# CityU-AIM-Group/MultiModal-learning

Measured on AMD Instinct MI355X. Metric: ROI-tiles/sec (teacher+student distill step), higher is better.
Workload: dtype bf16; 1 GPU; BASELINE configs[1]: teacher+student distill step, bf16, batch 64 per GPU, 512x512 tiles, 320-d omic, CRD P=300/K=700->P2=20/K2=512, n_data=1024, GK-Refine on, Adam+EMA, dropout 0.1; tiles_per_gpu=64, tile=512, global_batch=64, parallelism=single, launch=one captured HIP graph per step, input_pipeline=inputs resident in HBM when the timed region starts

## Files before the change

### multimodal-learning_amd/csrc/bn_act.hip

```cpp
#include "ph_common.h"
#include <cstdlib>
#include "ph_kernels.h"

namespace {

template <typename T>
__global__ void pack_input_kernel(const float* __restrict__ x, T* __restrict__ x4, int B, int H, int W) {
  const size_t npix = (size_t)B * H * W;
  const size_t i = (size_t)blockIdx.x * blockDim.x + threadIdx.x;
  if (i >= npix) return;
  const size_t hw = (size_t)H * W;
  const size_t b = i / hw, r = i - b * hw;
  const float c0 = x[(b * 3 + 0) * hw + r], c1 = x[(b * 3 + 1) * hw + r], c2 = x[(b * 3 + 2) * hw + r];
  if constexpr (is_hp<T>::value) {
    f16x4 h, l;
    f16 a, b;
    hp_split(c0, a, b); h[0] = a; l[0] = b;
    hp_split(c1, a, b); h[1] = a; l[1] = b;
    hp_split(c2, a, b); h[2] = a; l[2] = b;
    h[3] = (f16)0.f; l[3] = (f16)0.f;
    f16* base = reinterpret_cast<f16*>(x4);
    *reinterpret_cast<f16x4*>(base + i * 4) = h;
    *reinterpret_cast<f16x4*>(base + (npix + i) * 4) = l;
  } else if constexpr (is_f32<T>::value) {
// ... 42 lines not shown
  }
}

__global__ void bn_eval_params_kernel(PhBnEvalTable t, float eps) {
  const int u = blockIdx.x;
  for (int c = threadIdx.x; c < t.C[u]; c += blockDim.x) {
    const float is = rsqrtf(t.running_var[u][c] + eps);
    const float sc = t.gamma[u][c] * is;
    t.mean[u][c] = t.running_mean[u][c];
    t.invstd[u][c] = is;
    t.scale[u][c] = sc;
    t.shift[u][c] = t.beta[u][c] - t.running_mean[u][c] * sc;
  }
}

template <typename T, typename TY>
__global__ void bn_apply_kernel(const TY* __restrict__ y, const float* __restrict__ scale,
                                const float* __restrict__ shift, const TY* __restrict__ res,
                                const TY* __restrict__ y_r, const float* __restrict__ scale_r,
                                const float* __restrict__ shift_r, T* __restrict__ out, TY* __restrict__ out32, size_t n8,
                                int C8, int relu, int res_as_t) {
  const size_t i0 = (size_t)blockIdx.x * blockDim.x + threadIdx.x;
  if (i0 >= n8) return;
  const size_t gstride = (size_t)gridDim.x * blockDim.x;
  const int c = (int)(i0 % C8) * 8;
  const bool use_res = res != nullptr, use_yr = !use_res && y_r != nullptr;
  auto fetch = [&](size_t i, float (&v)[8], float (&r)[8]) {
    load8(y + i * 8, v);
    if (use_res) {
      if (!std::is_same<T, TY>::value && res_as_t) load8(reinterpret_cast<const T*>(res) + i * 8, r);
      else load8(res + i * 8, r);
    } else if (use_yr) {
      load8(y_r + i * 8, r);
    }
  };
  float v[8], r[8];
// ... 25 lines not shown
          const float t = __builtin_fmaf(r[k], scr8[k], shr8[k]);
          if constexpr (is_hp<T>::value) v[k] += (t > 0.f ? t : 0.f);
          else v[k] += (float)(T)(t > 0.f ? t : 0.f);
        }
      } else {
#pragma unroll
        for (int k = 0; k < 8; ++k) v[k] += r[k] * scr8[k] + shr8[k];
      }
    }
    if (relu & 1) {
#pragma unroll
      for (int k = 0; k < 8; ++k) v[k] = v[k] > 0.f ? v[k] : 0.f;
    }
    store8(out + i * 8, v);
    if constexpr (!std::is_same<T, TY>::value) { if (out32) store8(out32 + i * 8, v); }
    if (!more) break;
#pragma unroll
    for (int k = 0; k < 8; ++k) { v[k] = vn[k]; r[k] = rn[k]; }
    i = inext;
  }
}

template <typename T, typename TY, bool IDX>
__global__ void bn_relu_maxpool_kernel(const TY* __restrict__ y, const float* __restrict__ scale,
                                       const float* __restrict__ shift, T* __restrict__ out,
                                       uint8_t* __restrict__ idx, TY* __restrict__ raw, TY* __restrict__ out32, int B, int H,
                                       int W, int C8) {
  const int OH = (H + 1) / 2, OW = (W + 1) / 2;
  const size_t n = (size_t)B * OH * OW * C8;
  const size_t i = (size_t)blockIdx.x * blockDim.x + threadIdx.x;
// ... 116 lines not shown
  __device__ __forceinline__ void get(size_t i8, int c, float (&dz)[8], float (&yy)[8]) const {
    load8(g + i8 * 8, dz);
    load8(y + i8 * 8, yy);
    if (a) {
      float m[8];
      load8(a + i8 * 8, m);
#pragma unroll
      for (int k = 0; k < 8; ++k) dz[k] = m[k] > 0.f ? dz[k] : 0.f;
    } else if (mscale) {
#pragma unroll
      for (int k = 0; k < 8; ++k) dz[k] = __builtin_fmaf(yy[k], mscale[c + k], mshift[c + k]) > 0.f ? dz[k] : 0.f;
    }
  }
};

constexpr int BWD_BLOCKS_MAX = 1024;

template <typename T, typename Src>
__global__ __launch_bounds__(256) void bn_bwd_reduce_kernel(Src src, const float* __restrict__ mean,
                                                            const float* __restrict__ invstd,
                                                            float* __restrict__ parts, size_t npix, int C,
                                                            float* __restrict__ amax) {
  const int C8 = C >> 3;
  const int cg = threadIdx.x % C8, pl = threadIdx.x / C8, npl = 256 / C8;
  const int c = cg * 8;
  float mu[8], is[8], s1[8], s2[8], am = 0.f;
#pragma unroll
  for (int k = 0; k < 8; ++k) { s1[k] = 0.f; s2[k] = 0.f; }
  load8(mean + c, mu); load8(invstd + c, is);
  const size_t per = (npix + gridDim.x - 1) / gridDim.x;
// ... 362 lines not shown
  hipLaunchKernelGGL(bn_finalize_kernel, dim3(C), dim3(256), 0, st, parts, nparts, C, count, eps, momentum, gamma, beta,
                     mean, invstd, scale, shift, running_mean, running_var, nbt);
  PH_LAUNCH_CHECK();
  return PH_OK;
}

int ph_bn_eval_params_launch(const PhBnEvalTable* t, float eps, hipStream_t st) {
  hipLaunchKernelGGL(bn_eval_params_kernel, dim3(t->n), dim3(256), 0, st, *t, eps);
  PH_LAUNCH_CHECK();
  return PH_OK;
}

int ph_bn_apply_launch(const void* y, const float* scale, const float* shift, const void* res, const void* y_r,
                       const float* scale_r, const float* shift_r, void* out, void* out32, size_t npix, int C, int relu, int prec,
                       hipStream_t st) {
  return ph_bn_apply_launch2(y, scale, shift, res, y_r, scale_r, shift_r, out, out32, npix, C, relu, prec, 0, st);
}

int ph_bn_apply_launch2(const void* y, const float* scale, const float* shift, const void* res, const void* y_r,
                        const float* scale_r, const float* shift_r, void* out, void* out32, size_t npix, int C, int relu, int prec,
                        int res_as_t, hipStream_t st) {
  const size_t n8 = npix * (C / 8);
  void* tok = nullptr;
  if (ph_prof_on())
    ph_prof_begin(PH_CLS_BN_APPLY, (double)npix * C * (prec == PH_PREC_BF16 ? 2.0 : 4.0) * ((res || y_r) ? 3.0 : 2.0), st, &tok);
#define PH_CALL(T, TY)                                                                                              \
  hipLaunchKernelGGL((bn_apply_kernel<T, TY>), dim3(ew_grid(n8, C / 8)), dim3(256), 0, st, (const TY*)y, scale, shift, (const TY*)res, \
                     (const TY*)y_r, scale_r, shift_r, (T*)out, (TY*)out32, n8, C / 8, relu, res_as_t)
  PH_DISPATCH(prec, PH_CALL);
#undef PH_CALL
  ph_prof_end(tok, st);
  PH_LAUNCH_CHECK();
  return PH_OK;
}

int ph_bn_relu_maxpool_launch(const void* y, const float* scale, const float* shift, void* out, uint8_t* idx, void* raw,
                              void* out32, int B, int H, int W, int C, int prec, hipStream_t st) {
  const int OH = (H + 1) / 2, OW = (W + 1) / 2;
  const size_t n = (size_t)B * OH * OW * (C / 8);
#define PH_CALL(T, TY)                                                                                                          \
  do {                                                                                                                          \
    if (idx) hipLaunchKernelGGL((bn_relu_maxpool_kernel<T, TY, true>), dim3(nblk(n)), dim3(256), 0, st, (const TY*)y, scale, shift, \
                                (T*)out, idx, (TY*)raw, (TY*)out32, B, H, W, C / 8);                                            \
// ... 28 lines not shown
  const size_t n8 = (size_t)B * HW * (C / 8);
#define PH_CALL(T, TY) hipLaunchKernelGGL(avgpool_bwd_kernel<TY>, dim3(nblk(n8)), dim3(256), 0, st, g, (TY*)dx, n8, HW, C / 8, accumulate)
  PH_DISPATCH(prec, PH_CALL);
#undef PH_CALL
  PH_LAUNCH_CHECK();
  return PH_OK;
}

int ph_bn_bwd_parts(size_t npix, int C) {
  const size_t b = (npix * (size_t)(C / 8) + 2047) / 2048;
  return (int)(b < (size_t)BWD_BLOCKS_MAX ? (b ? b : 1) : BWD_BLOCKS_MAX);
}

int ph_bn_bwd_reduce_launch(const void* g, const void* a, const void* y, const float* mean, const float* invstd,
                            float* parts, size_t npix, int C, int prec, const float* mscale, const float* mshift,
                            float* amax, hipStream_t st) {
  const int nb = ph_bn_bwd_parts(npix, C);
#define PH_CALL(T, TY)                                                                                                       \
  do {                                                                                                                       \
    DzPlain<T, TY> s{(const TY*)g, (const TY*)a, (const TY*)y, mscale, mshift};                                              \
    hipLaunchKernelGGL((bn_bwd_reduce_kernel<T, DzPlain<T, TY>>), dim3(nb), dim3(256), 0, st, s, mean, invstd, parts, npix, C, amax); \
  } while (0)
  PH_DISPATCH(prec, PH_CALL);
#undef PH_CALL
  PH_LAUNCH_CHECK();
  return PH_OK;
}

int ph_bn_bwd_finalize_launch(const float* parts, int nparts, int C, double count, float* dgamma, float* dbeta,
                              float* c1, float* c2, const float* amax, int namax, const float* gamma, const float* invstd,
                              float* dzs, hipStream_t st) {
  hipLaunchKernelGGL(bn_bwd_finalize_kernel, dim3(C), dim3(256), 0, st, parts, nparts, C, count, dgamma, dbeta, c1, c2,
// ... 1 lines not shown
  PH_LAUNCH_CHECK();
  return PH_OK;
}

int ph_bn_bwd_finalize_fused_launch(const float* parts, int nparts, int C, double count, float* dgamma, float* dbeta,
                                    float* c1, float* c2, const float* invstd, int row2, hipStream_t st) {
  if (row2 != 1 && row2 != 2) return PH_EINVAL;
  hipLaunchKernelGGL(bn_bwd_finalize_kernel, dim3(C), dim3(256), 0, st, parts, nparts, C, count, dgamma, dbeta, c1, c2,
                     (const float*)nullptr, 0, (const float*)nullptr, invstd, (float*)nullptr, 3, row2, invstd);
  PH_LAUNCH_CHECK();
  return PH_OK;
}

int ph_bn_bwd_apply_launch(const void* g, const void* a, const void* y, const float* mean, const float* invstd,
                           const float* gamma, const float* c1, const float* c2, void* dy, size_t npix, int C,
                           int prec, const float* mscale, const float* mshift, const float* dzs, hipStream_t st) {
  const size_t n8 = npix * (C / 8);
#define PH_CALL(T, TY)                                                                                                       \
  do {                                                                                                                       \
    DzPlain<T, TY> s{(const TY*)g, (const TY*)a, (const TY*)y, mscale, mshift};                                              \
    hipLaunchKernelGGL((bn_bwd_apply_kernel<T, DzPlain<T, TY>>), dim3(ew_grid(n8, C / 8)), dim3(256), 0, st, s, mean, invstd, gamma, c1, c2, \
                       (T*)dy, n8, C / 8, dzs);                                                                              \
  } while (0)
  PH_DISPATCH(prec, PH_CALL);
#undef PH_CALL
  PH_LAUNCH_CHECK();
  return PH_OK;
}

int ph_stem_bwd_parts(int B, int H) { return (B * H + STEM_ROWS - 1) / STEM_ROWS; }

int ph_stem_bwd_reduce_launch(const void* dpool, const uint8_t* idx, const void* y0, const void* raw, const float* mean,
// ... 49 lines not shown
```

### multimodal-learning_amd/csrc/conv_wgrad.hip

```cpp
#include "ph_common.h"
#include "ph_kernels.h"

namespace {

__device__ __forceinline__ void lds_dma16(const void* g, unsigned lds_addr) {
  asm volatile("s_mov_b32 m0, %0\n\ts_nop 0\n\tglobal_load_lds_dwordx4 %1, off" : : "s"(lds_addr), "v"(g) : "memory");
}

__device__ __forceinline__ int sw_piece(int pix, int piece) { return piece ^ (((pix >> 1) & 1) << 1); }

template <typename T, int S, int TH, int KS>
struct WgCfg {
  static constexpr bool SPLIT = is_f32<T>::value;
  static constexpr bool HPM = is_hp<T>::value;
  static constexpr int TW = 16, BM = TH * TW;
  static constexpr int HPH = (TH - 1) * S + KS, HPW = (TW - 1) * S + KS, HP = HPH * HPW;
  static constexpr int HPP = (HP + 7) / 8 * 8;
  static constexpr int D_BYTES = BM * 128, X_BYTES = HPP * 128;
  static constexpr int NP = SPLIT ? PH_NPLANES : 1;
  static constexpr int LDS_BYTES = SPLIT ? (D_BYTES + X_BYTES) * NP : 2 * (D_BYTES + X_BYTES);
  static constexpr int NT = KS * KS;
};

template <typename T>
// ... 28 lines not shown
template <typename T, int S, int TH, int KS>
__global__ __launch_bounds__(256) void wgrad_kernel(PhWgrad p) {
  using C = WgCfg<T, S, TH, KS>;
  constexpr bool SPLIT = C::SPLIT, HPM = C::HPM;
  constexpr int TW = C::TW, BM = C::BM, HPW = C::HPW, HP = C::HP, NT = C::NT, NP = C::NP;
  typedef typename std::conditional<HPM, f16, T>::type TI;
  constexpr int EW = HPM ? 2 : 1;
  extern __shared__ __attribute__((aligned(16))) unsigned char smem[];
  unsigned char* ldsD = smem;
  unsigned char* ldsX = smem + C::D_BYTES * NP;

  const int tid = threadIdx.x, lane = tid & 63;
  const int wave = __builtin_amdgcn_readfirstlane(tid >> 6);
  const int cf = wave >> 1, kf = wave & 1;
  const int cin_blocks = p.Cin >> 6;
  const int co0 = (blockIdx.x / cin_blocks) << 6, ci0 = (blockIdx.x % cin_blocks) << 6;
  const int chunk = blockIdx.y;
  const int tiles_w = (p.OW + TW - 1) / TW, tiles_h = (p.OH + TH - 1) / TH;
  const int tiles_img = tiles_w * tiles_h, ntiles = tiles_img * p.B;
  const int t_begin = chunk * p.tiles_per_chunk;
  const int t_end = min(ntiles, t_begin + p.tiles_per_chunk);
  const TI* X = reinterpret_cast<const TI*>(p.x);
  const TI* DY = reinterpret_cast<const TI*>(p.dy);
  const long xpix = (p.x_pix_stride ? p.x_pix_stride : p.Cin) * EW;
  const long xrow = (p.x_row_stride ? p.x_row_stride : (long)p.IW * p.Cin) * EW;
  const long ximg = (p.x_img_stride ? p.x_img_stride : (long)p.IH * p.IW * p.Cin) * EW;
  const long dpix = (long)p.Cout * EW;

  f32x16 acc[NT];
#pragma unroll
  for (int t = 0; t < NT; ++t)
#pragma unroll
// ... 472 lines not shown
    }
    hipLaunchKernelGGL(pack_all_tiled_hp_kernel<false>, dim3(pt.tstart[t->n]), dim3(256), 0, st, *t, pt, (f16*)packed, 0);
  } else if (tiled && nplanes == 1)
    hipLaunchKernelGGL(pack_all_tiled_kernel<1>, dim3(pt.tstart[t->n]), dim3(256), 0, st, *t, pt, (bf16*)packed);
  else if (tiled && nplanes == 3)
    hipLaunchKernelGGL(pack_all_tiled_kernel<3>, dim3(pt.tstart[t->n]), dim3(256), 0, st, *t, pt, (bf16*)packed);
  else
    hipLaunchKernelGGL(pack_all_kernel, dim3((unsigned)((t->total + 255) / 256)), dim3(256), 0, st, *t, (bf16*)packed,
                       nplanes);
  PH_LAUNCH_CHECK();
  return PH_OK;
}

int ph_wgrad_tile_h(int S) { return S == 1 ? 8 : 4; }

int ph_wgrad_launch(const PhWgrad* p, int prec, hipStream_t st) {
  if (p->Cin % 64 || p->Cout % 64 || p->nchunks < 1) return PH_EINVAL;
  if (prec == PH_PREC_BF16) { ph_dispatch_note(PH_DK_WGRAD_BF16); return launch_wg_T<bf16>(*p, st); }
  if (prec == PH_PREC_FP16X3 || prec == PH_PREC_FP16X1) {
    PhWgrad q = *p;
    q.hp_hi_only = prec == PH_PREC_FP16X1;
    ph_dispatch_note(PH_DK_WGRAD_HP16);
    return launch_wg_T<hp16>(q, st);
  }
  if (PH_IS_SPLIT_PREC(prec)) {
    PhWgrad q = *p;
    q.prod6 = prec == PH_PREC_BF16X6;
    ph_dispatch_note(PH_DK_WGRAD_F32);
    return launch_wg_T<float>(q, st);
  }
  return PH_EINVAL;
}
// ... 30 lines not shown
```

### multimodal-learning_amd/csrc/ph_kernels.h

```cpp
#pragma once
#include <hip/hip_runtime.h>
#include <stdint.h>

#define PH_CLS_TAPCONV_N64 0
#define PH_CLS_TAPCONV_N128 1
#define PH_CLS_TAPCONV_S2 2
#define PH_CLS_WGRAD 3
#define PH_CLS_STEM_FWD 4
#define PH_CLS_STEM_WGRAD 5
#define PH_CLS_TAPCONV2 6
#define PH_CLS_TAPCONV2_RES 7
#define PH_CLS_CRD_SCORE 8
#define PH_CLS_CRD_LOSSGRAD 9
#define PH_CLS_ADAM_EMA 10
#define PH_CLS_BN_APPLY 11
#define PH_CLS_TAPCONV2_MASKED 12
#define PH_CLS_TAPCONV2_FUSEDIN 13
#define PH_CLS_TAPCONV2_RES_FUSEDIN 14
#define PH_CLS_CRD_TOPK 15
#define PH_NCLS 16
#define PH_NUM_CLS 6
bool ph_prof_on();
int ph_num_cus();
void ph_prof_begin(int cls, double work, hipStream_t st, void** token);
// ... 84 lines not shown
int ph_tapconv6b_launch(const PhTapConv* p, hipStream_t st);
int ph_tapconv6b_stat_parts(const PhTapConv* p);
bool ph_tapconv2_setup_s2_fwd(PhTapConv* t, int Cin, int Cout, int IH, int IW, int prec);

struct PhWgrad {
  const void* x;
  const void* dy;
  float* slab;
  const void* zeros;
  int B, IH, IW, Cin, OH, OW, Cout;
  int S, pad, KS;
  int nchunks, tiles_per_chunk;
  long x_pix_stride, x_row_stride, x_img_stride;
  int prod6;
  int hp_hi_only;
};
int ph_wgrad_launch(const PhWgrad* p, int prec, hipStream_t st);
int ph_wgrad_tile_h(int S);
int ph_wgrad_reduce_launch(const float* slab, float* dw_oihw, int nchunks, int KS, int Cout, int Cin, const float* unscale,
                           hipStream_t st);

struct PhStem {
  const void* x4;
  const void* w;
  size_t wplane;
  void* out;
  float* stats;
  int B, IH, IW, OH, OW;
  int prod6;
  int vblocks;
};
// ... 40 lines not shown
                          float* shift, float* running_mean, float* running_var, int64_t* num_batches_tracked,
                          hipStream_t st);
struct PhBnEvalTable {
  const float* gamma[20]; const float* beta[20]; const float* running_mean[20]; const float* running_var[20];
  float* mean[20]; float* invstd[20]; float* scale[20]; float* shift[20];
  int C[20];
  int n;
};
int ph_bn_eval_params_launch(const PhBnEvalTable* t, float eps, hipStream_t st);
int ph_bn_apply_launch(const void* y, const float* scale, const float* shift, const void* res, const void* y_r,
                       const float* scale_r, const float* shift_r, void* out, void* out32, size_t npix, int C, int relu, int prec,
                       hipStream_t st);
int ph_bn_apply_launch2(const void* y, const float* scale, const float* shift, const void* res, const void* y_r,
                        const float* scale_r, const float* shift_r, void* out, void* out32, size_t npix, int C, int relu, int prec,
                        int res_as_t, hipStream_t st);
int ph_avgpool_launch_t(const void* x, float* out, int B, int HW, int C, int prec, hipStream_t st);
int ph_bn_relu_maxpool_launch(const void* y, const float* scale, const float* shift, void* out, uint8_t* idx, void* raw,
                              void* out32, int B, int H, int W, int C, int prec, hipStream_t st);
int ph_avgpool_launch(const void* x, float* out, int B, int HW, int C, int prec, hipStream_t st);
int ph_avgpool_bwd_launch(const float* g, void* dx, int B, int HW, int C, int accumulate, int prec, hipStream_t st);
int ph_bn_bwd_parts(size_t npix, int C);
int ph_stem_bwd_parts(int B, int H);
int ph_bn_bwd_reduce_launch(const void* g, const void* a, const void* y, const float* mean, const float* invstd,
                            float* parts, size_t npix, int C, int prec, const float* mscale, const float* mshift,
                            float* amax, hipStream_t st);
int ph_bn_bwd_finalize_launch(const float* parts, int nparts, int C, double count, float* dgamma, float* dbeta,
                              float* c1, float* c2, const float* amax, int namax, const float* gamma, const float* invstd,
                              float* dzs, hipStream_t st);
int ph_bn_bwd_finalize_fused_launch(const float* parts, int nparts, int C, double count, float* dgamma, float* dbeta,
                                    float* c1, float* c2, const float* invstd, int row2, hipStream_t st);
int ph_bn_bwd_apply_launch(const void* g, const void* a, const void* y, const float* mean, const float* invstd,
                           const float* gamma, const float* c1, const float* c2, void* dy, size_t npix, int C,
                           int prec, const float* mscale, const float* mshift, const float* dzs, hipStream_t st);
int ph_stem_bwd_reduce_launch(const void* dpool, const uint8_t* idx, const void* y0, const void* raw_at_argmax, const float* mean,
                              const float* invstd, const float* scale, const float* shift, float* parts, int B, int H,
                              int W, int C, int prec, float* amax, hipStream_t st);
int ph_stem_bwd_apply_launch(const void* dpool, const uint8_t* idx, const void* y0, const float* mean,
                             const float* invstd, const float* scale, const float* shift, const float* gamma,
                             const float* c1, const float* c2, void* dy0, int B, int H, int W, int C, int prec,
                             const float* dzs, hipStream_t st);
```

### multimodal-learning_amd/csrc/resnet_plan.hip

```cpp
#include <atomic>
#include <cstdlib>
#include <iterator>
#include <mutex>
#include <new>
#include <unordered_map>
#include <vector>
#include "ph_common.h"
#include "ph_kernels.h"
#include "ph_dense.h"

namespace {

struct Unit {
  int Cin, Cout, KS, S, pad;
  int IH, IW, OH, OW;
  size_t wf_off, wd_off;
  size_t wplane;
  size_t y_off;
  size_t st_off;
  mutable int wfrag_f = 0, wfrag_d = 0;
};

void fwd_geometry(const Unit& u, PhTapConv& t) {
  t.IH = u.IH; t.IW = u.IW; t.Cin = u.Cin; t.Cout = u.Cout;
// ... 3 lines not shown
}
void dgrad_s1_geometry(const Unit& u, PhTapConv& t) {
  t.IH = u.OH; t.IW = u.OW; t.Cin = u.Cout; t.Cout = u.Cin;
  t.OH = u.IH; t.OW = u.IW;
  t.OHt = u.IH; t.OWt = u.IW; t.os = 1; t.oa_h = 0; t.oa_w = 0;
  t.iy0 = -(u.KS - 1 - u.pad); t.ix0 = t.iy0; t.ntaps = u.KS * u.KS;
  for (int k = 0; k < t.ntaps; ++k) {
    const int dyy = k / u.KS, dxx = k % u.KS;
    t.dy[k] = dyy; t.dx[k] = dxx; t.wtap[k] = (u.KS - 1 - dyy) * u.KS + (u.KS - 1 - dxx);
  }
}
struct Block {
  int u1, u2, uds;
  size_t in_off, a1_off, out_off;
  size_t in32_off, out32_off;
  int IH, IW, OH, OW, Cin, Cout;
};

constexpr size_t ALIGN = 256;
inline size_t up(size_t x) { return (x + ALIGN - 1) / ALIGN * ALIGN; }

}

struct PhResnetPlan {
  int B, H, W, prec, es;
  std::vector<Unit> units;
  std::vector<Block> blocks;
  size_t x4_off, p0_off, p0raw_off, idx_off, parts_off, parts_bytes;
  size_t g0_off, g1_off, dy_off, da_off, slab_off, slab_bytes, bparts_off, cc_off, zero_off;
  size_t ws_bytes, packed_bytes;
// ... 129 lines not shown
  P->slab_off = take(slab_max);
  {
    const size_t stem_rows = (size_t)ph_stem_bwd_parts(B, s.OH);
    const size_t a = (size_t)1024 * 2 * 512, b = stem_rows * 2 * 64;
    P->bparts_off = take((a > b ? a : b) * sizeof(float));
  }
  P->cc_off = take(2 * 512 * sizeof(float));
  P->zero_off = take(256);
  {
    const size_t rows = std::max((size_t)1024, (size_t)ph_stem_bwd_parts(B, s.OH));
    P->amax_off = take(rows * sizeof(float));
    P->dzs_off = take(256);
  }
  P->fparts_off = take((size_t)1024 * 3 * 512 * sizeof(float));
  P->cc2_off = take(2 * 512 * sizeof(float));
  P->ws_bytes = off;
  P->packed_bytes = woff * sizeof(bf16);
  refresh_layouts(P);
  return P;
}

void ph_resnet_plan_destroy(PhResnetPlan* P) { delete P; }
size_t ph_resnet_workspace_bytes(const PhResnetPlan* P) { return P ? P->ws_bytes : 0; }
size_t ph_resnet_packed_bytes(const PhResnetPlan* P) { return P ? P->packed_bytes : 0; }
int ph_resnet_num_units(const PhResnetPlan* P) { return P ? (int)P->units.size() : 0; }
int ph_resnet_unit_shape(const PhResnetPlan* P, int u, int* out4) {
  if (!P || u < 0 || u >= (int)P->units.size()) return PH_EINVAL;
  out4[0] = P->units[u].Cout; out4[1] = P->units[u].Cin; out4[2] = P->units[u].KS; out4[3] = P->units[u].S;
  return PH_OK;
}
// ... 64 lines not shown
  }
  int rc = ph_tapconv_launch(&t, S, P->prec, c.st);
  if (rc || c.eval) return rc;
  const int nparts = ph_tapconv_stat_parts(&t, S, P->prec);
  float* rm = c.update_running ? (float*)c.params[ui * 6 + 3] : nullptr;
  return ph_bn_finalize_launch(t.stats, nparts, u.Cout, (double)P->B * u.OH * u.OW, 1e-5f, 0.1f,
                               (const float*)c.params[ui * 6 + 1], (const float*)c.params[ui * 6 + 2], c.stat(u, 0),
                               c.stat(u, 1), c.stat(u, 2), c.stat(u, 3), rm, (float*)c.params[ui * 6 + 4],
                               (int64_t*)c.params[ui * 6 + 5], c.st);
}

struct Bst { int u = -1, u2 = -1; const void* a = nullptr; };

int bst_switch(int set) {
  static int on = [] { const char* e = getenv("PH_BST"); return (e && e[0] == '0') ? 0 : 1; }();
  if (set >= 0) on = set ? 1 : 0;
  return on;
}

int conv_dgrad(const Ctx& c, int ui, const void* dy, void* dx, const void* res_g, const void* res_a, const float* dzs = nullptr,
               const Bst* bst = nullptr, int* fused_parts = nullptr) {
  const PhResnetPlan* P = c.P;
  const Unit& u = P->units[ui];
  PhTapConv t{};
  t.in = dy; t.w = c.pk + u.wd_off; t.wplane = u.wplane; t.in_unscale = dzs;
  t.out = dx; t.stats = nullptr; t.res_g = res_g; t.res_a = res_a;
  t.B = P->B; t.IH = u.OH; t.IW = u.OW; t.Cin = u.Cout; t.Cout = u.Cin;
  t.OH = u.IH; t.OW = u.IW;
  t.w_frag = u.wfrag_d;
  if (fused_parts) *fused_parts = 0;
// ... 81 lines not shown
  w.x = x; w.dy = dy; w.slab = reinterpret_cast<float*>(c.ws + P->slab_off);
  w.zeros = c.ws + P->zero_off;
  w.B = P->B; w.IH = u.IH; w.IW = u.IW; w.Cin = u.Cin; w.OH = u.OH; w.OW = u.OW; w.Cout = u.Cout;
  w.S = u.S; w.pad = u.pad; w.KS = u.KS;
  if (u.KS == 1 && u.S == 2) {
    w.x_pix_stride = 2L * u.Cin; w.x_row_stride = 2L * u.IW * u.Cin; w.x_img_stride = (long)u.IH * u.IW * u.Cin;
    w.IH = u.OH; w.IW = u.OW; w.S = 1;
  }
  w.nchunks = wgrad_chunks(u, P->B, &w.tiles_per_chunk, c.wg_want);
  int rc = ph_wgrad_launch(&w, c.bprec(), c.st);
  if (rc) return rc;
  return ph_wgrad_reduce_launch(w.slab, dw, w.nchunks, u.KS, u.Cout, u.Cin, dzs, c.st);
}

int bn_bwd(const Ctx& c, int ui, const void* g, const void* a, void* dy, float* dgamma, float* dbeta, bool self_mask = false,
           float* dzs = nullptr, int fused_parts = 0, int row2 = 1, bool cc2 = false, bool finalize = true, bool apply = true) {
  const PhResnetPlan* P = c.P;
  const Unit& u = P->units[ui];
  const size_t npix = (size_t)P->B * u.OH * u.OW;
  float* parts = reinterpret_cast<float*>(c.ws + P->bparts_off);
  float* c1 = reinterpret_cast<float*>(c.ws + (cc2 ? P->cc2_off : P->cc_off));
  float* c2 = c1 + 512;
  const void* y = c.ws + u.y_off;
  const float* ms = self_mask ? c.stat(u, 2) : nullptr;
  const float* mh = self_mask ? c.stat(u, 3) : nullptr;
  if (self_mask) a = nullptr;
  float* amax = dzs ? c.amax() : nullptr;
  int rc = PH_OK;
  if (finalize) {
    if (fused_parts > 0) {
      rc = ph_bn_bwd_finalize_fused_launch(reinterpret_cast<const float*>(c.ws + P->fparts_off), fused_parts, u.Cout, (double)npix,
                                           dgamma, dbeta, c1, c2, c.stat(u, 1), row2, c.st);
    } else {
      const int nparts = ph_bn_bwd_parts(npix, u.Cout);
      rc = ph_bn_bwd_reduce_launch(g, a, y, c.stat(u, 0), c.stat(u, 1), parts, npix, u.Cout, P->prec, ms, mh, amax, c.st);
      if (rc) return rc;
      rc = ph_bn_bwd_finalize_launch(parts, nparts, u.Cout, (double)npix, dgamma, dbeta, c1, c2, amax, nparts,
                                     (const float*)c.params[ui * 6 + 1], c.stat(u, 1), dzs, c.st);
    }
    if (rc) return rc;
  }
  if (!apply) return PH_OK;
  return ph_bn_bwd_apply_launch(g, a, y, c.stat(u, 0), c.stat(u, 1), (const float*)c.params[ui * 6 + 1], c1, c2, dy, npix,
                                u.Cout, P->prec, ms, mh, dzs, c.st);
}

}

extern "C" {

int ph_resnet_forward(const PhResnetPlan* P, const void* const* params, const void* packed, const float* x_nchw,
                      void* ws_, float* f3, float* f4, int flags, hipStream_t st) {
  if (!P || !params || !packed || !x_nchw || !ws_) return PH_EINVAL;
  Ctx c{P, params, reinterpret_cast<const bf16*>(packed), reinterpret_cast<unsigned char*>(ws_), st,
        (flags & 2) ? 0 : (flags & 1), (flags & 2) ? 1 : 0};
  P->no_masked = (flags & 16) ? 1 : 0;
  c.no_masked = P->no_masked;
  unsigned char* ws = c.ws;
  const bool hp = P->prec == PH_PREC_FP16X3;
// ... 57 lines not shown
                                    (int64_t*)params[5], st)))
      return rc;
    if ((rc = ph_bn_relu_maxpool_launch(ws + u.y_off, c.stat(u, 2), c.stat(u, 3), ws + P->p0_off,
                                        (flags & 4) ? nullptr : ws + P->idx_off, (flags & 4) ? nullptr : ws + P->p0raw_off,
                                        (hp && !fo_hp) ? ws + P->blocks[0].in32_off : nullptr, P->B, u.OH, u.OW, 64, P->prec, st)))
      return rc;
  }
  const bool fuse_a1 = (flags & 4) && !(flags & 8) && P->prec == PH_PREC_BF16;
  for (size_t bi = 0; bi < P->blocks.size(); ++bi) {
    const Block& b = P->blocks[bi];
    const Unit& u1 = P->units[b.u1];
    const Unit& u2 = P->units[b.u2];
    const size_t npix = (size_t)P->B * b.OH * b.OW;
    const Unit& u0 = P->units[0];
    const bool raw_in = bi == 0 && p0_raw;
    if ((rc = raw_in ? conv_fwd(c, b.u1, ws + b.in_off, c.stat(u0, 2), c.stat(u0, 3)) : conv_fwd(c, b.u1, ws + b.in_off))) return rc;
    static const bool fuse_all = [] { const char* e = getenv("PH_FUSE_ALL"); return e && e[0] == '1'; }();
    if (fuse_a1 && (b.Cout <= 128 || fuse_all)) {
      if ((rc = conv_fwd(c, b.u2, ws + u1.y_off, c.stat(u1, 2), c.stat(u1, 3)))) return rc;
    } else {
      if ((rc = ph_bn_apply_launch(ws + u1.y_off, c.stat(u1, 2), c.stat(u1, 3), nullptr, nullptr, nullptr, nullptr,
                                   ws + b.a1_off, nullptr, npix, b.Cout, 1, P->prec, st)))
        return rc;
      if ((rc = conv_fwd(c, b.u2, ws + b.a1_off))) return rc;
    }
    if (b.uds >= 0) {
      const Unit& ud = P->units[b.uds];
      if ((rc = conv_fwd(c, b.uds, ws + b.in_off))) return rc;
      rc = ph_bn_apply_launch(ws + u2.y_off, c.stat(u2, 2), c.stat(u2, 3), nullptr, ws + ud.y_off, c.stat(ud, 2),
                              c.stat(ud, 3), ws + b.out_off, (hp && !fo_hp) ? ws + b.out32_off : nullptr, npix, b.Cout, 1, P->prec, st);
    } else {
      rc = raw_in ? ph_bn_apply_launch(ws + u2.y_off, c.stat(u2, 2), c.stat(u2, 3), nullptr, ws + b.in_off, c.stat(u0, 2),
                                       c.stat(u0, 3), ws + b.out_off, nullptr, npix, b.Cout, 3, P->prec, st)
                  : ph_bn_apply_launch2(ws + u2.y_off, c.stat(u2, 2), c.stat(u2, 3), fo_hp ? ws + b.in_off : ws + b.in32_off, nullptr,
                                        nullptr, nullptr, ws + b.out_off, (hp && !fo_hp) ? ws + b.out32_off : nullptr, npix, b.Cout, 1,
                                        P->prec, fo_hp ? 1 : 0, st);
    }
    if (rc) return rc;
    if ((bi == 5 && f3) || (bi == 7 && f4)) {
      float* dst = bi == 5 ? f3 : f4;
      if ((rc = fo_hp ? ph_avgpool_launch_t(ws + b.out_off, dst, P->B, b.OH * b.OW, b.Cout, P->prec, st)
                      : ph_avgpool_launch(ws + b.out32_off, dst, P->B, b.OH * b.OW, b.Cout, P->prec, st)))
        return rc;
    }
  }
  return PH_OK;
}

}

namespace {
// ... 127 lines not shown
  if (part != 1) {
    if (hipMemsetAsync(ws + P->zero_off, 0, 256, st) != hipSuccess) return PH_ELAUNCH;
    const Block& b = P->blocks[7];
    PH_STAGE(ph_avgpool_bwd_launch(g_f4, gcur, P->B, b.OH * b.OW, b.Cout, 0, P->prec, st));
  }
  for (int bi = bi_hi; bi >= bi_lo; --bi) {
    const Block& b = P->blocks[bi];
    if (bi == 5 && g_f3) {
      PH_STAGE(ph_avgpool_bwd_launch(g_f3, gcur, P->B, b.OH * b.OW, b.Cout, 1, P->prec, st));
      fused_out = 0;
    }
    const void* out = ws + b.out32_off;
    const void* a1 = ws + b.a1_off;
    const void* xin = ws + b.in_off;
    const void* xin32 = ws + b.in32_off;
    if ((rc = claim(k))) return rc;
    if (fused_out > 0 && b.uds >= 0 &&
        (rc = bn_bwd(c, b.uds, gcur, out, nullptr, (float*)grads[b.uds * 3 + 1], (float*)grads[b.uds * 3 + 2], false, nullptr,
                     fused_out, 2, true, true, false)))
      return rc;
    const bool ds_done = fused_out > 0 && b.uds >= 0;
    PH_STAGE(bn_bwd(c, b.u2, gcur, out, dzb[k], (float*)grads[b.u2 * 3 + 1], (float*)grads[b.u2 * 3 + 2], false, c.dzs(k), fused_out));
    fused_out = 0;
    if (!ov) PH_STAGE(wgrad_of(b.u2, a1, k));
    int fused_a1 = 0;
    {
      Bst bs; bs.u = b.u1;
      PH_STAGE(conv_dgrad(c, b.u2, dzb[k], dab, nullptr, nullptr, c.dzs(k), &bs, &fused_a1));
    }
    if (ov) PH_STAGE(wgrad_of(b.u2, a1, k));
    k ^= 1;
    if ((rc = claim(k))) return rc;
    PH_STAGE(bn_bwd(c, b.u1, dab, a1, dzb[k], (float*)grads[b.u1 * 3 + 1], (float*)grads[b.u1 * 3 + 2], true, c.dzs(k), fused_a1));
    if (!ov) PH_STAGE(wgrad_of(b.u1, xin, k));
    if (b.uds < 0) {
      Bst bs;
      if (bi > bi_lo) {
        const Block& pb = P->blocks[bi - 1];
        bs.u = pb.u2; bs.u2 = pb.uds; bs.a = xin32;
      }
        PH_STAGE(conv_dgrad(c, b.u1, dzb[k], gnext, gcur, out, c.dzs(k), &bs, &fused_out));
      if (ov) PH_STAGE(wgrad_of(b.u1, xin, k));
      k ^= 1;
    } else {
        PH_STAGE(conv_dgrad(c, b.u1, dzb[k], gnext, nullptr, nullptr, c.dzs(k)));
      if (ov) PH_STAGE(wgrad_of(b.u1, xin, k));
      k ^= 1;
      if ((rc = claim(k))) return rc;
      PH_STAGE(bn_bwd(c, b.uds, gcur, out, dzb[k], (float*)grads[b.uds * 3 + 1], (float*)grads[b.uds * 3 + 2], false, c.dzs(k),
                      0, 1, ds_done, !ds_done));
      if (!ov) PH_STAGE(wgrad_of(b.uds, xin, k));
        PH_STAGE(conv_dgrad(c, b.uds, dzb[k], gnext, gnext, nullptr, c.dzs(k)));
      if (ov) PH_STAGE(wgrad_of(b.uds, xin, k));
      k ^= 1;
    }
    unsigned char* t = gcur; gcur = gnext; gnext = t;
  }
  if (part != 0) {
    const Unit& u = P->units[0];
    const size_t npix = (size_t)P->B * u.OH * u.OW;
    float* parts = reinterpret_cast<float*>(ws + P->bparts_off);
    float* c1 = reinterpret_cast<float*>(ws + P->cc_off);
    float* c2 = c1 + 512;
    if ((rc = ph_stem_bwd_reduce_launch(gcur, ws + P->idx_off, ws + u.y_off, ws + P->p0raw_off, c.stat(u, 0), c.stat(u, 1),
                                        c.stat(u, 2), c.stat(u, 3), parts, P->B, u.OH, u.OW, 64, P->prec, c.amax(), st)))
// ... 32 lines not shown

}

extern "C" {

unsigned long long ph_resnet_plan_layout_sig(const PhResnetPlan* P) { return P ? refresh_layouts(P) : 0; }

int ph_resnet_plan_set_backward_prec(const PhResnetPlan* P, int prec) {
  if (!P || (prec != -1 && P->prec == PH_PREC_BF16)) return PH_EINVAL;
  if (prec != -1 && !(P->prec == PH_PREC_FP16X3 ? (prec == PH_PREC_FP16X1 || prec == PH_PREC_FP16X3) : PH_IS_SPLIT_PREC(prec))) return PH_EINVAL;
  P->bwd_prec = prec;
  return PH_OK;
}

int ph_debug_set_bst(int on) { return bst_switch(on ? 1 : 0); }

int ph_resnet_plan_set_backward_overlap(const PhResnetPlan* P, int on) {
  if (!P) return PH_EINVAL;
  P->bwd_overlap = on ? 1 : 0;
  return PH_OK;
}

int ph_pack_input(const float* x_nchw, void* x4, int B, int H, int W, int prec, hipStream_t st) {
  if (!x_nchw || !x4 || B < 1 || H < 1 || W < 1 || (prec != PH_PREC_BF16 && !PH_IS_SPLIT_PREC(prec) && prec != PH_PREC_FP16X3))
    return PH_EINVAL;
  return ph_pack_input_launch(x_nchw, x4, B, H, W, prec, st);
}

int ph_resnet_backward(const PhResnetPlan* P, const void* const* params, const void* packed, void* ws_,
                       const float* g_f3, const float* g_f4, void* const* grads, hipStream_t st) {
// ... 18 lines not shown
  Ctx c{P, params, reinterpret_cast<const bf16*>(packed), reinterpret_cast<unsigned char*>(ws_), st, 0, 1};
  c.no_masked = P->no_masked;
  unsigned char* ws = c.ws;
  unsigned char* gcur = ws + P->g0_off;
  unsigned char* gnext = ws + P->g1_off;
  unsigned char* dyb = ws + P->dy_off;
  unsigned char* dab = ws + P->da_off;
  float* c1 = reinterpret_cast<float*>(ws + P->cc_off);
  float* c2 = c1 + 512;
  int rc;
  if (hipMemsetAsync(ws + P->zero_off, 0, 256, st) != hipSuccess) return PH_ELAUNCH;
  if (hipMemsetAsync(c1, 0, 1024 * sizeof(float), st) != hipSuccess) return PH_ELAUNCH;
  auto bn_eval_bwd = [&](int ui, const void* g, const void* a, void* dy) -> int {
    const Unit& u = P->units[ui];
    return ph_bn_bwd_apply_launch(g, a, ws + u.y_off, c.stat(u, 0), c.stat(u, 1), (const float*)params[ui * 6 + 1], c1, c2,
                                  dy, (size_t)P->B * u.OH * u.OW, u.Cout, P->prec, nullptr, nullptr, nullptr, st);
  };
  {
    const Block& b = P->blocks[7];
    if ((rc = ph_avgpool_bwd_launch(g_f4, gcur, P->B, b.OH * b.OW, b.Cout, 0, P->prec, st))) return rc;
  }
  for (int bi = 7; bi >= 0; --bi) {
    const Block& b = P->blocks[bi];
    if (bi == 5 && g_f3)
      if ((rc = ph_avgpool_bwd_launch(g_f3, gcur, P->B, b.OH * b.OW, b.Cout, 1, P->prec, st))) return rc;
    const void* out = ws + b.out_off;
    const void* a1 = ws + b.a1_off;
    if ((rc = bn_eval_bwd(b.u2, gcur, out, dyb))) return rc;
    if ((rc = conv_dgrad(c, b.u2, dyb, dab, nullptr, nullptr))) return rc;
    if ((rc = bn_eval_bwd(b.u1, dab, a1, dyb))) return rc;
    if (b.uds < 0) {
// ... 30 lines not shown
    return PH_OK;
  }
  if (what >= 4 && what <= 7) {
    *byte_off = what == 4 ? P->g0_off : what == 5 ? P->g1_off : what == 6 ? P->dy_off : P->da_off;
    dims4[0] = dims4[1] = dims4[2] = dims4[3] = 0;
    return PH_OK;
  }
  if (what == 8 && id >= 0 && id < (int)P->units.size()) {
    *byte_off = P->units[id].st_off; dims4[0] = 4; dims4[1] = P->units[id].Cout; dims4[2] = dims4[3] = 1;
    return PH_OK;
  }
  if (what == 9) {
    *byte_off = P->idx_off; dims4[0] = P->B; dims4[1] = P->PH0; dims4[2] = P->PW0; dims4[3] = 64;
    return PH_OK;
  }
  return PH_EINVAL;
}

}
```

Baseline: 6447 tiles/s.

## Store ReLU masks as bitfields and remap wgrad workgroups across XCDs

```diff
diff --git a/multimodal-learning_amd/csrc/bn_act.hip b/multimodal-learning_amd/csrc/bn_act.hip
--- a/multimodal-learning_amd/csrc/bn_act.hip
+++ b/multimodal-learning_amd/csrc/bn_act.hip
@@ -80,12 +80,12 @@
   }
 }
 
-template <typename T, typename TY>
+template <typename T, typename TY, bool BITS = false>
 __global__ void bn_apply_kernel(const TY* __restrict__ y, const float* __restrict__ scale,
                                 const float* __restrict__ shift, const TY* __restrict__ res,
                                 const TY* __restrict__ y_r, const float* __restrict__ scale_r,
                                 const float* __restrict__ shift_r, T* __restrict__ out, TY* __restrict__ out32, size_t n8,
-                                int C8, int relu, int res_as_t) {
+                                int C8, int relu, int res_as_t, uint8_t* __restrict__ bits) {
   const size_t i0 = (size_t)blockIdx.x * blockDim.x + threadIdx.x;
   if (i0 >= n8) return;
   const size_t gstride = (size_t)gridDim.x * blockDim.x;
@@ -141,6 +141,17 @@
     }
     store8(out + i * 8, v);
     if constexpr (!std::is_same<T, TY>::value) { if (out32) store8(out32 + i * 8, v); }
+    if constexpr (BITS) {
+      unsigned m = 0;
+#pragma unroll
+      for (int k = 0; k < 8; ++k) {
+        bool pos;
+        if constexpr (std::is_same<T, TY>::value && !is_f32<T>::value) pos = (float)(T)v[k] > 0.f;
+        else pos = v[k] > 0.f;
+        m |= (pos ? 1u : 0u) << k;
+      }
+      bits[i] = (uint8_t)m;
+    }
     if (!more) break;
 #pragma unroll
     for (int k = 0; k < 8; ++k) { v[k] = vn[k]; r[k] = rn[k]; }
@@ -287,6 +298,25 @@
   }
 };
 
+template <typename T, typename TY = T>
+struct DzBits {
+  const TY* g; const uint8_t* bits; const TY* y;
+  static constexpr const TY* a = nullptr;
+  static constexpr const float* mscale = nullptr;
+  static constexpr const float* mshift = nullptr;
+  __device__ __forceinline__ void fetch(size_t i8, float (&dz)[8], float (&yy)[8], float (&m)[8]) const {
+    load8(g + i8 * 8, dz);
+    load8(y + i8 * 8, yy);
+    m[0] = (float)bits[i8];
+  }
+  __device__ __forceinline__ void mask(const float (&)[8], const float (&)[8], float (&dz)[8], const float (&)[8],
+                                       const float (&m)[8]) const {
+    const unsigned b = (unsigned)m[0];
+#pragma unroll
+    for (int k = 0; k < 8; ++k) dz[k] = ((b >> k) & 1u) ? dz[k] : 0.f;
+  }
+};
+
 constexpr int BWD_BLOCKS_MAX = 1024;
 
 template <typename T, typename Src>
@@ -679,19 +709,31 @@
 int ph_bn_apply_launch(const void* y, const float* scale, const float* shift, const void* res, const void* y_r,
                        const float* scale_r, const float* shift_r, void* out, void* out32, size_t npix, int C, int relu, int prec,
                        hipStream_t st) {
-  return ph_bn_apply_launch2(y, scale, shift, res, y_r, scale_r, shift_r, out, out32, npix, C, relu, prec, 0, st);
+  return ph_bn_apply_launch3(y, scale, shift, res, y_r, scale_r, shift_r, out, out32, npix, C, relu, prec, 0, nullptr, st);
 }
 
 int ph_bn_apply_launch2(const void* y, const float* scale, const float* shift, const void* res, const void* y_r,
                         const float* scale_r, const float* shift_r, void* out, void* out32, size_t npix, int C, int relu, int prec,
                         int res_as_t, hipStream_t st) {
+  return ph_bn_apply_launch3(y, scale, shift, res, y_r, scale_r, shift_r, out, out32, npix, C, relu, prec, res_as_t, nullptr, st);
+}
+
+int ph_bn_apply_launch3(const void* y, const float* scale, const float* shift, const void* res, const void* y_r,
+                        const float* scale_r, const float* shift_r, void* out, void* out32, size_t npix, int C, int relu, int prec,
+                        int res_as_t, uint8_t* bits, hipStream_t st) {
   const size_t n8 = npix * (C / 8);
+  if (bits && prec == PH_PREC_FP16X3 && !out32) return PH_EINVAL;
   void* tok = nullptr;
   if (ph_prof_on())
-    ph_prof_begin(PH_CLS_BN_APPLY, (double)npix * C * (prec == PH_PREC_BF16 ? 2.0 : 4.0) * ((res || y_r) ? 3.0 : 2.0), st, &tok);
+    ph_prof_begin(PH_CLS_BN_APPLY,
+                  (double)npix * C * (prec == PH_PREC_BF16 ? 2.0 : 4.0) * ((res || y_r) ? 3.0 : 2.0) + (bits ? (double)n8 : 0.0), st, &tok);
 #define PH_CALL(T, TY)                                                                                              \
-  hipLaunchKernelGGL((bn_apply_kernel<T, TY>), dim3(ew_grid(n8, C / 8)), dim3(256), 0, st, (const TY*)y, scale, shift, (const TY*)res, \
-                     (const TY*)y_r, scale_r, shift_r, (T*)out, (TY*)out32, n8, C / 8, relu, res_as_t)
+  do {                                                                                                              \
+    if (bits) hipLaunchKernelGGL((bn_apply_kernel<T, TY, true>), dim3(ew_grid(n8, C / 8)), dim3(256), 0, st, (const TY*)y, scale, shift, \
+                                 (const TY*)res, (const TY*)y_r, scale_r, shift_r, (T*)out, (TY*)out32, n8, C / 8, relu, res_as_t, bits); \
+    else hipLaunchKernelGGL((bn_apply_kernel<T, TY, false>), dim3(ew_grid(n8, C / 8)), dim3(256), 0, st, (const TY*)y, scale, shift, \
+                            (const TY*)res, (const TY*)y_r, scale_r, shift_r, (T*)out, (TY*)out32, n8, C / 8, relu, res_as_t, bits); \
+  } while (0)
   PH_DISPATCH(prec, PH_CALL);
 #undef PH_CALL
   ph_prof_end(tok, st);
@@ -750,8 +792,19 @@
 
 int ph_bn_bwd_reduce_launch(const void* g, const void* a, const void* y, const float* mean, const float* invstd,
                             float* parts, size_t npix, int C, int prec, const float* mscale, const float* mshift,
-                            float* amax, hipStream_t st) {
+                            float* amax, const uint8_t* bits, hipStream_t st) {
   const int nb = ph_bn_bwd_parts(npix, C);
+  if (bits) {
+#define PH_CALL(T, TY)                                                                                                       \
+  do {                                                                                                                       \
+    DzBits<T, TY> s{(const TY*)g, bits, (const TY*)y};                                                                       \
+    hipLaunchKernelGGL((bn_bwd_reduce_kernel<T, DzBits<T, TY>>), dim3(nb), dim3(256), 0, st, s, mean, invstd, parts, npix, C, amax); \
+  } while (0)
+    PH_DISPATCH(prec, PH_CALL);
+#undef PH_CALL
+    PH_LAUNCH_CHECK();
+    return PH_OK;
+  }
 #define PH_CALL(T, TY)                                                                                                       \
   do {                                                                                                                       \
     DzPlain<T, TY> s{(const TY*)g, (const TY*)a, (const TY*)y, mscale, mshift};                                              \
@@ -783,8 +836,21 @@
 
 int ph_bn_bwd_apply_launch(const void* g, const void* a, const void* y, const float* mean, const float* invstd,
                            const float* gamma, const float* c1, const float* c2, void* dy, size_t npix, int C,
-                           int prec, const float* mscale, const float* mshift, const float* dzs, hipStream_t st) {
+                           int prec, const float* mscale, const float* mshift, const float* dzs, const uint8_t* bits,
+                           hipStream_t st) {
   const size_t n8 = npix * (C / 8);
+  if (bits) {
+#define PH_CALL(T, TY)                                                                                                       \
+  do {                                                                                                                       \
+    DzBits<T, TY> s{(const TY*)g, bits, (const TY*)y};                                                                       \
+    hipLaunchKernelGGL((bn_bwd_apply_kernel<T, DzBits<T, TY>>), dim3(ew_grid(n8, C / 8)), dim3(256), 0, st, s, mean, invstd, gamma, c1, c2, \
+                       (T*)dy, n8, C / 8, dzs);                                                                              \
+  } while (0)
+    PH_DISPATCH(prec, PH_CALL);
+#undef PH_CALL
+    PH_LAUNCH_CHECK();
+    return PH_OK;
+  }
 #define PH_CALL(T, TY)                                                                                                       \
   do {                                                                                                                       \
     DzPlain<T, TY> s{(const TY*)g, (const TY*)a, (const TY*)y, mscale, mshift};                                              \
diff --git a/multimodal-learning_amd/csrc/conv_wgrad.hip b/multimodal-learning_amd/csrc/conv_wgrad.hip
--- a/multimodal-learning_amd/csrc/conv_wgrad.hip
+++ b/multimodal-learning_amd/csrc/conv_wgrad.hip
@@ -1,4 +1,5 @@
 #include "ph_common.h"
+#include <cstdlib>
 #include "ph_kernels.h"
 
 namespace {
@@ -66,8 +67,10 @@
   const int wave = __builtin_amdgcn_readfirstlane(tid >> 6);
   const int cf = wave >> 1, kf = wave & 1;
   const int cin_blocks = p.Cin >> 6;
-  const int co0 = (blockIdx.x / cin_blocks) << 6, ci0 = (blockIdx.x % cin_blocks) << 6;
-  const int chunk = blockIdx.y;
+  unsigned wg_block, wg_chunk;
+  ph_wgrad_map(blockIdx.y * gridDim.x + blockIdx.x, gridDim.x, gridDim.y, (unsigned)cin_blocks, p.xcd, &wg_block, &wg_chunk);
+  const int co0 = (int)(wg_block / (unsigned)cin_blocks) << 6, ci0 = (int)(wg_block % (unsigned)cin_blocks) << 6;
+  const int chunk = (int)wg_chunk;
   const int tiles_w = (p.OW + TW - 1) / TW, tiles_h = (p.OH + TH - 1) / TH;
   const int tiles_img = tiles_w * tiles_h, ntiles = tiles_img * p.B;
   const int t_begin = chunk * p.tiles_per_chunk;
@@ -570,8 +573,17 @@
 
 int ph_wgrad_tile_h(int S) { return S == 1 ? 8 : 4; }
 
-int ph_wgrad_launch(const PhWgrad* p, int prec, hipStream_t st) {
-  if (p->Cin % 64 || p->Cout % 64 || p->nchunks < 1) return PH_EINVAL;
+int ph_wg_xcd_switch(int set) {
+  static int on = [] { const char* e = getenv("PH_WG_XCD"); return (e && e[0] == '0') ? 0 : 1; }();
+  if (set >= 0) on = set ? 1 : 0;
+  return on;
+}
+
+int ph_wgrad_launch(const PhWgrad* p_, int prec, hipStream_t st) {
+  if (p_->Cin % 64 || p_->Cout % 64 || p_->nchunks < 1) return PH_EINVAL;
+  PhWgrad pv = *p_;
+  pv.xcd = ph_wg_xcd_switch(-1);
+  const PhWgrad* p = &pv;
   if (prec == PH_PREC_BF16) { ph_dispatch_note(PH_DK_WGRAD_BF16); return launch_wg_T<bf16>(*p, st); }
   if (prec == PH_PREC_FP16X3 || prec == PH_PREC_FP16X1) {
     PhWgrad q = *p;
diff --git a/multimodal-learning_amd/csrc/ph_kernels.h b/multimodal-learning_amd/csrc/ph_kernels.h
--- a/multimodal-learning_amd/csrc/ph_kernels.h
+++ b/multimodal-learning_amd/csrc/ph_kernels.h
@@ -122,7 +122,18 @@
   long x_pix_stride, x_row_stride, x_img_stride;
   int prod6;
   int hp_hi_only;
-};
+  int xcd;
+};
+__host__ __device__ inline void ph_wgrad_map(unsigned id, unsigned blocks, unsigned nchunks, unsigned cin_blocks, int xcd,
+                                             unsigned* block, unsigned* chunk) {
+  if (!xcd) { *block = id % blocks; *chunk = id / blocks; return; }
+  const unsigned nwg = blocks * nchunks, q = nwg >> 3, r = nwg & 7u, x = id & 7u;
+  const unsigned w = (x < r ? x * (q + 1) : r * (q + 1) + (x - r) * q) + (id >> 3);
+  const unsigned j = w % blocks, cout_blocks = blocks / cin_blocks;
+  *chunk = w / blocks;
+  *block = (j % cout_blocks) * cin_blocks + j / cout_blocks;
+}
+int ph_wg_xcd_switch(int set);
 int ph_wgrad_launch(const PhWgrad* p, int prec, hipStream_t st);
 int ph_wgrad_tile_h(int S);
 int ph_wgrad_reduce_launch(const float* slab, float* dw_oihw, int nchunks, int KS, int Cout, int Cin, const float* unscale,
@@ -193,6 +204,9 @@
 int ph_bn_apply_launch2(const void* y, const float* scale, const float* shift, const void* res, const void* y_r,
                         const float* scale_r, const float* shift_r, void* out, void* out32, size_t npix, int C, int relu, int prec,
                         int res_as_t, hipStream_t st);
+int ph_bn_apply_launch3(const void* y, const float* scale, const float* shift, const void* res, const void* y_r,
+                        const float* scale_r, const float* shift_r, void* out, void* out32, size_t npix, int C, int relu, int prec,
+                        int res_as_t, uint8_t* bits, hipStream_t st);
 int ph_avgpool_launch_t(const void* x, float* out, int B, int HW, int C, int prec, hipStream_t st);
 int ph_bn_relu_maxpool_launch(const void* y, const float* scale, const float* shift, void* out, uint8_t* idx, void* raw,
                               void* out32, int B, int H, int W, int C, int prec, hipStream_t st);
@@ -202,7 +216,7 @@
 int ph_stem_bwd_parts(int B, int H);
 int ph_bn_bwd_reduce_launch(const void* g, const void* a, const void* y, const float* mean, const float* invstd,
                             float* parts, size_t npix, int C, int prec, const float* mscale, const float* mshift,
-                            float* amax, hipStream_t st);
+                            float* amax, const uint8_t* bits, hipStream_t st);
 int ph_bn_bwd_finalize_launch(const float* parts, int nparts, int C, double count, float* dgamma, float* dbeta,
                               float* c1, float* c2, const float* amax, int namax, const float* gamma, const float* invstd,
                               float* dzs, hipStream_t st);
@@ -210,7 +224,8 @@
                                     float* c1, float* c2, const float* invstd, int row2, hipStream_t st);
 int ph_bn_bwd_apply_launch(const void* g, const void* a, const void* y, const float* mean, const float* invstd,
                            const float* gamma, const float* c1, const float* c2, void* dy, size_t npix, int C,
-                           int prec, const float* mscale, const float* mshift, const float* dzs, hipStream_t st);
+                           int prec, const float* mscale, const float* mshift, const float* dzs, const uint8_t* bits,
+                           hipStream_t st);
 int ph_stem_bwd_reduce_launch(const void* dpool, const uint8_t* idx, const void* y0, const void* raw_at_argmax, const float* mean,
                               const float* invstd, const float* scale, const float* shift, float* parts, int B, int H,
                               int W, int C, int prec, float* amax, hipStream_t st);
diff --git a/multimodal-learning_amd/csrc/resnet_plan.hip b/multimodal-learning_amd/csrc/resnet_plan.hip
--- a/multimodal-learning_amd/csrc/resnet_plan.hip
+++ b/multimodal-learning_amd/csrc/resnet_plan.hip
@@ -41,6 +41,7 @@
   int u1, u2, uds;
   size_t in_off, a1_off, out_off;
   size_t in32_off, out32_off;
+  size_t bits_off;
   int IH, IW, OH, OW, Cin, Cout;
 };
 
@@ -200,6 +201,7 @@
   }
   P->fparts_off = take((size_t)1024 * 3 * 512 * sizeof(float));
   P->cc2_off = take(2 * 512 * sizeof(float));
+  for (Block& b : P->blocks) b.bits_off = take((size_t)B * b.OH * b.OW * b.Cout / 8);
   P->ws_bytes = off;
   P->packed_bytes = woff * sizeof(bf16);
   refresh_layouts(P);
@@ -294,6 +296,12 @@
 
 int bst_switch(int set) {
   static int on = [] { const char* e = getenv("PH_BST"); return (e && e[0] == '0') ? 0 : 1; }();
+  if (set >= 0) on = set ? 1 : 0;
+  return on;
+}
+
+int mask_bits_switch(int set) {
+  static int on = [] { const char* e = getenv("PH_MASK_BITS"); return (e && e[0] == '0') ? 0 : 1; }();
   if (set >= 0) on = set ? 1 : 0;
   return on;
 }
@@ -405,7 +413,8 @@
 }
 
 int bn_bwd(const Ctx& c, int ui, const void* g, const void* a, void* dy, float* dgamma, float* dbeta, bool self_mask = false,
-           float* dzs = nullptr, int fused_parts = 0, int row2 = 1, bool cc2 = false, bool finalize = true, bool apply = true) {
+           float* dzs = nullptr, int fused_parts = 0, int row2 = 1, bool cc2 = false, bool finalize = true, bool apply = true,
+           const uint8_t* bits = nullptr) {
   const PhResnetPlan* P = c.P;
   const Unit& u = P->units[ui];
   const size_t npix = (size_t)P->B * u.OH * u.OW;
@@ -415,7 +424,8 @@
   const void* y = c.ws + u.y_off;
   const float* ms = self_mask ? c.stat(u, 2) : nullptr;
   const float* mh = self_mask ? c.stat(u, 3) : nullptr;
-  if (self_mask) a = nullptr;
+  if (self_mask) { a = nullptr; bits = nullptr; }
+  if (bits) a = nullptr;
   float* amax = dzs ? c.amax() : nullptr;
   int rc = PH_OK;
   if (finalize) {
@@ -424,7 +434,7 @@
                                            dgamma, dbeta, c1, c2, c.stat(u, 1), row2, c.st);
     } else {
       const int nparts = ph_bn_bwd_parts(npix, u.Cout);
-      rc = ph_bn_bwd_reduce_launch(g, a, y, c.stat(u, 0), c.stat(u, 1), parts, npix, u.Cout, P->prec, ms, mh, amax, c.st);
+      rc = ph_bn_bwd_reduce_launch(g, a, y, c.stat(u, 0), c.stat(u, 1), parts, npix, u.Cout, P->prec, ms, mh, amax, bits, c.st);
       if (rc) return rc;
       rc = ph_bn_bwd_finalize_launch(parts, nparts, u.Cout, (double)npix, dgamma, dbeta, c1, c2, amax, nparts,
                                      (const float*)c.params[ui * 6 + 1], c.stat(u, 1), dzs, c.st);
@@ -433,7 +443,7 @@
   }
   if (!apply) return PH_OK;
   return ph_bn_bwd_apply_launch(g, a, y, c.stat(u, 0), c.stat(u, 1), (const float*)c.params[ui * 6 + 1], c1, c2, dy, npix,
-                                u.Cout, P->prec, ms, mh, dzs, c.st);
+                                u.Cout, P->prec, ms, mh, dzs, bits, c.st);
 }
 
 }
@@ -521,6 +531,7 @@
     const size_t npix = (size_t)P->B * b.OH * b.OW;
     const Unit& u0 = P->units[0];
     const bool raw_in = bi == 0 && p0_raw;
+    uint8_t* const bits = (!(flags & 4) && mask_bits_switch(-1)) ? ws + b.bits_off : nullptr;
     if ((rc = raw_in ? conv_fwd(c, b.u1, ws + b.in_off, c.stat(u0, 2), c.stat(u0, 3)) : conv_fwd(c, b.u1, ws + b.in_off))) return rc;
     static const bool fuse_all = [] { const char* e = getenv("PH_FUSE_ALL"); return e && e[0] == '1'; }();
     if (fuse_a1 && (b.Cout <= 128 || fuse_all)) {
@@ -534,14 +545,15 @@
     if (b.uds >= 0) {
       const Unit& ud = P->units[b.uds];
       if ((rc = conv_fwd(c, b.uds, ws + b.in_off))) return rc;
-      rc = ph_bn_apply_launch(ws + u2.y_off, c.stat(u2, 2), c.stat(u2, 3), nullptr, ws + ud.y_off, c.stat(ud, 2),
-                              c.stat(ud, 3), ws + b.out_off, (hp && !fo_hp) ? ws + b.out32_off : nullptr, npix, b.Cout, 1, P->prec, st);
+      rc = ph_bn_apply_launch3(ws + u2.y_off, c.stat(u2, 2), c.stat(u2, 3), nullptr, ws + ud.y_off, c.stat(ud, 2),
+                               c.stat(ud, 3), ws + b.out_off, (hp && !fo_hp) ? ws + b.out32_off : nullptr, npix, b.Cout, 1, P->prec, 0,
+                               bits, st);
     } else {
       rc = raw_in ? ph_bn_apply_launch(ws + u2.y_off, c.stat(u2, 2), c.stat(u2, 3), nullptr, ws + b.in_off, c.stat(u0, 2),
                                        c.stat(u0, 3), ws + b.out_off, nullptr, npix, b.Cout, 3, P->prec, st)
-                  : ph_bn_apply_launch2(ws + u2.y_off, c.stat(u2, 2), c.stat(u2, 3), fo_hp ? ws + b.in_off : ws + b.in32_off, nullptr,
+                  : ph_bn_apply_launch3(ws + u2.y_off, c.stat(u2, 2), c.stat(u2, 3), fo_hp ? ws + b.in_off : ws + b.in32_off, nullptr,
                                         nullptr, nullptr, ws + b.out_off, (hp && !fo_hp) ? ws + b.out32_off : nullptr, npix, b.Cout, 1,
-                                        P->prec, fo_hp ? 1 : 0, st);
+                                        P->prec, fo_hp ? 1 : 0, bits, st);
     }
     if (rc) return rc;
     if ((bi == 5 && f3) || (bi == 7 && f4)) {
@@ -699,13 +711,15 @@
     const void* a1 = ws + b.a1_off;
     const void* xin = ws + b.in_off;
     const void* xin32 = ws + b.in32_off;
+    const uint8_t* obits = mask_bits_switch(-1) ? ws + b.bits_off : nullptr;
     if ((rc = claim(k))) return rc;
     if (fused_out > 0 && b.uds >= 0 &&
         (rc = bn_bwd(c, b.uds, gcur, out, nullptr, (float*)grads[b.uds * 3 + 1], (float*)grads[b.uds * 3 + 2], false, nullptr,
-                     fused_out, 2, true, true, false)))
+                     fused_out, 2, true, true, false, obits)))
       return rc;
     const bool ds_done = fused_out > 0 && b.uds >= 0;
-    PH_STAGE(bn_bwd(c, b.u2, gcur, out, dzb[k], (float*)grads[b.u2 * 3 + 1], (float*)grads[b.u2 * 3 + 2], false, c.dzs(k), fused_out));
+    PH_STAGE(bn_bwd(c, b.u2, gcur, out, dzb[k], (float*)grads[b.u2 * 3 + 1], (float*)grads[b.u2 * 3 + 2], false, c.dzs(k), fused_out, 1, false,
+                    true, true, obits));
     fused_out = 0;
     if (!ov) PH_STAGE(wgrad_of(b.u2, a1, k));
     int fused_a1 = 0;
@@ -733,7 +747,7 @@
       k ^= 1;
       if ((rc = claim(k))) return rc;
       PH_STAGE(bn_bwd(c, b.uds, gcur, out, dzb[k], (float*)grads[b.uds * 3 + 1], (float*)grads[b.uds * 3 + 2], false, c.dzs(k),
-                      0, 1, ds_done, !ds_done));
+                      0, 1, ds_done, !ds_done, true, obits));
       if (!ov) PH_STAGE(wgrad_of(b.uds, xin, k));
         PH_STAGE(conv_dgrad(c, b.uds, dzb[k], gnext, gnext, nullptr, c.dzs(k)));
       if (ov) PH_STAGE(wgrad_of(b.uds, xin, k));
@@ -796,6 +810,24 @@
 }
 
 int ph_debug_set_bst(int on) { return bst_switch(on ? 1 : 0); }
+int ph_debug_set_mask_bits(int on) { return mask_bits_switch(on ? 1 : 0); }
+int ph_debug_set_wg_xcd(int on) { return ph_wg_xcd_switch(on ? 1 : 0); }
+int ph_debug_wgrad_map(int id, int blocks, int nchunks, int cin_blocks, int xcd, int* block, int* chunk) {
+  if (id < 0 || blocks < 1 || nchunks < 1 || cin_blocks < 1 || blocks % cin_blocks || id >= blocks * nchunks || !block || !chunk) return PH_EINVAL;
+  unsigned b, c;
+  ph_wgrad_map((unsigned)id, (unsigned)blocks, (unsigned)nchunks, (unsigned)cin_blocks, xcd, &b, &c);
+  *block = (int)b; *chunk = (int)c;
+  return PH_OK;
+}
+int ph_debug_wgrad_grid(const PhResnetPlan* P, int u, int beside, int* blocks, int* nchunks, int* cin_blocks) {
+  if (!P || u < 1 || u >= (int)P->units.size() || !blocks || !nchunks || !cin_blocks) return PH_EINVAL;
+  const Unit& un = P->units[u];
+  int tpc;
+  *nchunks = wgrad_chunks(un, P->B, &tpc, beside ? WG_WANT_BESIDE : WG_WANT_ALONE);
+  *blocks = (un.Cout / 64) * (un.Cin / 64);
+  *cin_blocks = un.Cin / 64;
+  return PH_OK;
+}
 
 int ph_resnet_plan_set_backward_overlap(const PhResnetPlan* P, int on) {
   if (!P) return PH_EINVAL;
@@ -844,7 +876,7 @@
   auto bn_eval_bwd = [&](int ui, const void* g, const void* a, void* dy) -> int {
     const Unit& u = P->units[ui];
     return ph_bn_bwd_apply_launch(g, a, ws + u.y_off, c.stat(u, 0), c.stat(u, 1), (const float*)params[ui * 6 + 1], c1, c2,
-                                  dy, (size_t)P->B * u.OH * u.OW, u.Cout, P->prec, nullptr, nullptr, nullptr, st);
+                                  dy, (size_t)P->B * u.OH * u.OW, u.Cout, P->prec, nullptr, nullptr, nullptr, nullptr, st);
   };
   {
     const Block& b = P->blocks[7];
@@ -905,6 +937,16 @@
     *byte_off = P->idx_off; dims4[0] = P->B; dims4[1] = P->PH0; dims4[2] = P->PW0; dims4[3] = 64;
     return PH_OK;
   }
+  if (what == 11 && id >= 0 && id < (int)P->blocks.size()) {
+    const Block& b = P->blocks[id];
+    *byte_off = b.out32_off; dims4[0] = P->B; dims4[1] = b.OH; dims4[2] = b.OW; dims4[3] = b.Cout;
+    return PH_OK;
+  }
+  if (what == 10 && id >= 0 && id < (int)P->blocks.size()) {
+    const Block& b = P->blocks[id];
+    *byte_off = b.bits_off; dims4[0] = P->B; dims4[1] = b.OH; dims4[2] = b.OW; dims4[3] = b.Cout;
+    return PH_OK;
+  }
   return PH_EINVAL;
 }
 
```

New measurement: 6576 tiles/s, median of 4. 2.0% higher.
